# imazen/codec-eval

Measured on AMD Instinct MI355X. Metric: metric MP/s (SSIMULACRA2+DSSIM+Butteraugli) at 1/2/4/8 GPU; HBM-roofline %, higher is better.
Workload: dtype f32

## Files before the change

### codec-eval_amd/csrc/butteraugli.hip

```cpp
#include <algorithm>
#include <cmath>
#include <cstdlib>
#include <type_traits>

#include "ce_internal.h"

namespace {

constexpr int TPB = 256;
constexpr int PSY = 10;
enum { UHF0 = 0, UHF1, HF0, HF1, MF0, MF1, MF2, LF0, LF1, LF2 };

struct geom {
    uint32_t w, h, pitch;
    size_t plane;
};

struct blur_kernel {
    int len;
    float k[40];
    float lo[16], hi[16];
};

#define BA_XY                                                           \
    const uint32_t x = blockIdx.x * 64 + (threadIdx.x & 63);            \
    const uint32_t y = blockIdx.y * 4 + (threadIdx.x >> 6);             \
    if (x >= g.w || y >= g.h) return;                                   \
    const size_t o = (size_t)y * g.pitch + x

__device__ __forceinline__ uint32_t slot_of(uint32_t z, uint32_t n_refs_used, uint32_t max_refs)
{
    return z < n_refs_used ? z : max_refs + (z - n_refs_used);
}

struct plane_sel {
    uint32_t per_unit, first, n;
};

__device__ __forceinline__ uint32_t mirror(int x, int n)
{
    while (x < 0 || x >= n) x = x < 0 ? -x - 1 : 2 * n - 1 - x;
    return (uint32_t)x;
}

constexpr int BW_OUT = 8;

#ifndef CE_BA_BLUR_FMA
#define CE_BA_BLUR_FMA 0
#endif
__device__ __forceinline__ float blur_tap(float sum, float v, float k)
{
#if CE_BA_BLUR_FMA
    return __builtin_fmaf(v, k, sum);
#else
    return sum + v * k;
#endif
}

template <int LEN>
__device__ __forceinline__ float border_scale(const blur_kernel &bk, int pos, int n, float inv_wsum)
{
    constexpr int off = LEN / 2;
    if (pos - off >= 0 && pos + off <= n - 1) return inv_wsum;
    if (n >= LEN) {
        const int d = pos < off ? pos : n - 1 - pos;
        float s = 0.0f;
#pragma unroll
        for (int i = 0; i < off; i++) s = d == i ? (pos < off ? bk.lo[i] : bk.hi[i]) : s;
        return s;
    }
    float weight = 0.0f;
    for (int j = max(pos - off, 0); j <= min(pos + off, n - 1); j++) weight += bk.k[j - pos + off];
    return 1.0f / weight;
}

typedef float ba_f2 __attribute__((ext_vector_type(2)));
#ifndef CE_BH_TILES
#define CE_BH_TILES 4
#endif
constexpr int BH_TILES = CE_BH_TILES;

template <int LEN>
__global__ __launch_bounds__(TPB) void k_ba_blur_h(const float *__restrict__ in, float *__restrict__ out, geom g, plane_sel si,
                                                   plane_sel so, blur_kernel bk, float inv_wsum, uint32_t n_refs_used,
                                                   uint32_t max_refs, int by_slot, uint32_t z0)
{
    constexpr int off = LEN / 2, TW = 256, TR = 8, LEFT = 16, RAW = TW + 2 * LEFT, ROWF = RAW + RAW / 8 + 1, SH = LEFT - off;
    static_assert(off <= LEFT, "tile halo");
    __shared__ float tile[TR * ROWF];
    const uint32_t u = blockIdx.z / si.n + z0, k = blockIdx.z % si.n;
    const uint32_t unit = by_slot ? slot_of(u, n_refs_used, max_refs) : u;
    const float *p = in + ((size_t)unit * si.per_unit + si.first + k) * g.plane;
    const int x0 = blockIdx.x * TW;
    constexpr int NF = (TR * (RAW / 4) + TPB - 1) / TPB;
    float4 pf[NF];
    auto fetch = [&](int y0) {
#pragma unroll
        for (int m = 0; m < NF; m++) {
            const int i = m * TPB + (int)threadIdx.x, r = i / (RAW / 4), c = 4 * (i % (RAW / 4)), gx = x0 - LEFT + c, gy = y0 + r;
            float4 v = make_float4(0.0f, 0.0f, 0.0f, 0.0f);
            if (r < TR && gx >= 0 && gx < (int)g.pitch && gy < (int)g.h) {
                v = *reinterpret_cast<const float4 *>(p + (size_t)gy * g.pitch + gx);
                if (gx + 3 >= (int)g.w) {
                    if (gx + 0 >= (int)g.w) v.x = 0.0f;
                    if (gx + 1 >= (int)g.w) v.y = 0.0f;
                    if (gx + 2 >= (int)g.w) v.z = 0.0f;
                    v.w = 0.0f;
                }
            }
            pf[m] = v;
        }
    };
    const int r = threadIdx.x >> 5, cx = threadIdx.x & 31, gx0 = x0 + 8 * cx;
    __shared__ __attribute__((aligned(16))) float s_scale[TW];
    {
        const int gx = x0 + (int)threadIdx.x;
        s_scale[threadIdx.x] = gx < (int)g.w ? border_scale<LEN>(bk, gx, (int)g.w, inv_wsum) : 0.0f;
    }
    constexpr int NV = BW_OUT + LEN - 1, NP = (NV + 1) / 2;
    const float *row = &tile[r * ROWF + 9 * cx];
    auto at = [&](int j) { return row[(j + SH) + ((j + SH) >> 3)]; };
    const int y_first = blockIdx.y * (TR * BH_TILES);
    fetch(y_first);
#pragma unroll 1
    for (int t = 0; t < BH_TILES; t++) {
        const int y0 = y_first + t * TR;
        if (y0 >= (int)g.h) break;
        if (t) __syncthreads();
#pragma unroll
        for (int m = 0; m < NF; m++) {
            const int i = m * TPB + (int)threadIdx.x, rr = i / (RAW / 4), c = 4 * (i % (RAW / 4));
            if (rr < TR) {
                float *tp = &tile[rr * ROWF + c + (c >> 3)];
                tp[0] = pf[m].x, tp[1] = pf[m].y, tp[2] = pf[m].z, tp[3] = pf[m].w;
            }
        }
        if (t + 1 < BH_TILES && y0 + TR < (int)g.h) fetch(y0 + TR);
        __syncthreads();
        const int gy = y0 + r;
        if (gy >= (int)g.h || gx0 >= (int)g.w) continue;
        ba_f2 pe[NP], po[NP];
#pragma unroll
        for (int i = 0; i < NP; i++) {
            pe[i] = ba_f2{at(2 * i), 2 * i + 1 < NV ? at(2 * i + 1) : 0.0f};
            po[i] = ba_f2{2 * i + 1 < NV ? at(2 * i + 1) : 0.0f, 2 * i + 2 < NV ? at(2 * i + 2) : 0.0f};
        }
        float *dst = out + ((size_t)unit * so.per_unit + so.first + k) * g.plane + (size_t)gy * g.pitch + gx0;
        float res[BW_OUT];
#pragma unroll
        for (int op = 0; op < BW_OUT / 2; op++) {
            ba_f2 sum = {0.0f, 0.0f};
#pragma unroll
            for (int j = 0; j < LEN; j++) {
                const int idx = 2 * op + j;
                const ba_f2 src = (idx & 1) ? po[idx >> 1] : pe[idx >> 1];
#if CE_BA_BLUR_FMA
                sum = __builtin_elementwise_fma(src, ba_f2{bk.k[j], bk.k[j]}, sum);
#else
                const ba_f2 prod = src * ba_f2{bk.k[j], bk.k[j]};
                sum = sum + prod;
#endif
            }
            res[2 * op] = sum.x * s_scale[8 * cx + 2 * op];
            res[2 * op + 1] = sum.y * s_scale[8 * cx + 2 * op + 1];
        }
        if (gx0 + BW_OUT <= (int)g.w) {
            *reinterpret_cast<float4 *>(dst) = make_float4(res[0], res[1], res[2], res[3]);
            *reinterpret_cast<float4 *>(dst + 4) = make_float4(res[4], res[5], res[6], res[7]);
        } else {
#pragma unroll
            for (int o = 0; o < BW_OUT; o++)
                if (gx0 + o < (int)g.w) dst[o] = res[o];
        }
    }
}

__device__ __forceinline__ void opsin_absorbance(float in0, float in1, float in2, float &o0, float &o1, float &o2)
{
    const float mixi0 = 0.29956550340058319f, mixi1 = 0.63373087833825936f, mixi2 = 0.077705617820981968f, mixi3 = 1.7557483643287353f;
    const float mixi4 = 0.22158691104574774f, mixi5 = 0.69391388044116142f, mixi6 = 0.0987313588422f, mixi7 = 1.7557483643287353f;
    const float mixi8 = 0.02f, mixi9 = 0.02f, mixi10 = 0.20480129041026129f, mixi11 = 12.226454707163354f;
    o0 = __builtin_fmaf(mixi0, in0, __builtin_fmaf(mixi1, in1, __builtin_fmaf(mixi2, in2, mixi3)));
    o1 = __builtin_fmaf(mixi4, in0, __builtin_fmaf(mixi5, in1, __builtin_fmaf(mixi6, in2, mixi7)));
    o2 = __builtin_fmaf(mixi8, in0, __builtin_fmaf(mixi9, in1, __builtin_fmaf(mixi10, in2, mixi11)));
}

__device__ __forceinline__ float fast_log2f(float x)
{
    const float p0 = -1.8503833400518310E-06f, p1 = 1.4287160470083755E+00f, p2 = 7.4245873327820566E-01f;
    const float q0 = 9.9032814277590719E-01f, q1 = 1.0096718572241148E+00f, q2 = 1.7409343003366853E-01f;
    const int32_t xb = (int32_t)__float_as_uint(x);
    const int32_t es = (xb - 0x3f2aaaab) >> 23;
    const float m = __uint_as_float((uint32_t)xb - ((uint32_t)es << 23));
    const float t = m - 1.0f;
    const float yp = __builtin_fmaf(__builtin_fmaf(p2, t, p1), t, p0);
    const float yq = __builtin_fmaf(__builtin_fmaf(q2, t, q1), t, q0);
    return ce_div_noscale(yp, yq) + (float)es;
}

__device__ __forceinline__ float gamma_f(float v)
{
    const float kRetMul = 19.245013259874995f * 0.693147180559945f, kRetAdd = -23.16046239805755f;
    if (v < 0.0f) v = 0.0f;
    const float biased = v + 9.9710635769299145f;
    return __builtin_fmaf(kRetMul, fast_log2f(biased), kRetAdd);
}

constexpr int FT = 32, FR = FT + 4;
template <typename T>
__device__ __forceinline__ float ba_linear_of(const float *tab, T v) { return tab[v]; }
template <>
__device__ __forceinline__ float ba_linear_of<float>(const float *, float v) { return v; }

template <bool HALF, typename T>
__global__ __launch_bounds__(TPB) void k_ba_front(const uint8_t *__restrict__ refs, const uint8_t *__restrict__ tests,
                                                  const float *__restrict__ lut, const float *__restrict__ lut_test, geom gi,
                                                  float *__restrict__ xyb, geom g, float w0, float w1, float w2,
                                                  float intensity_target, size_t img_bytes, uint32_t n_refs_used, uint32_t max_refs,
                                                  uint32_t z0)
{
    __shared__ float L[3][FR * FR];
    __shared__ float H[3][FR * FT];
    constexpr bool U8 = sizeof(T) == 1;
    __shared__ float s_lut[256];
    if (U8) s_lut[threadIdx.x] = lut[threadIdx.x];
    const uint32_t z = blockIdx.z + z0, slot = slot_of(z, n_refs_used, max_refs);
    const int w = (int)g.w, h = (int)g.h, x0 = blockIdx.x * FT, y0 = blockIdx.y * FT, gx0 = x0 - 2, gy0 = y0 - 2;
    const uint8_t *src8 = z < n_refs_used ? refs + (size_t)z * img_bytes : tests + (size_t)(z - n_refs_used) * img_bytes;
    const T *srcT = reinterpret_cast<const T *>(src8);
    const float *tab = U8 ? s_lut : (z < n_refs_used ? lut : lut_test);
    const int W8 = HALF ? (int)gi.w : w, H8 = HALF ? (int)gi.h : h;
    __syncthreads();
    const bool interior = gx0 >= 0 && gy0 >= 0 && gx0 + FR <= w && gy0 + FR <= h;
    auto load12 = [&](const uint8_t *p, uint32_t &v0, uint32_t &v1, uint32_t &v2) {
        const uintptr_t a = reinterpret_cast<uintptr_t>(p);
        const uint32_t *q = reinterpret_cast<const uint32_t *>(a & ~(uintptr_t)3);
        const uint32_t d0 = q[0], d1 = q[1], d2 = q[2], d3 = q[3], sh = (uint32_t)(a & 3);
        v0 = __builtin_amdgcn_alignbyte(d1, d0, sh), v1 = __builtin_amdgcn_alignbyte(d2, d1, sh), v2 = __builtin_amdgcn_alignbyte(d3, d2, sh);
    };
    if (U8 && !HALF && interior) {
        for (int i = threadIdx.x; i < FR * (FR / 4); i += TPB) {
            const int ly = i / (FR / 4), lx = 4 * (i % (FR / 4));
            uint32_t v0, v1, v2;
            load12(src8 + ((size_t)(gy0 + ly) * w + gx0 + lx) * 3, v0, v1, v2);
            const int o = ly * FR + lx;
            L[0][o] = s_lut[v0 & 255u], L[1][o] = s_lut[(v0 >> 8) & 255u], L[2][o] = s_lut[(v0 >> 16) & 255u];
            L[0][o + 1] = s_lut[v0 >> 24], L[1][o + 1] = s_lut[v1 & 255u], L[2][o + 1] = s_lut[(v1 >> 8) & 255u];
            L[0][o + 2] = s_lut[(v1 >> 16) & 255u], L[1][o + 2] = s_lut[v1 >> 24], L[2][o + 2] = s_lut[v2 & 255u];
            L[0][o + 3] = s_lut[(v2 >> 8) & 255u], L[1][o + 3] = s_lut[(v2 >> 16) & 255u], L[2][o + 3] = s_lut[v2 >> 24];
        }
    } else if (U8 && HALF && interior && 2 * (gx0 + FR) <= W8 && 2 * (gy0 + FR) <= H8) {
        for (int i = threadIdx.x; i < FR * (FR / 2); i += TPB) {
            const int ly = i / (FR / 2), lx = 2 * (i % (FR / 2));
            uint32_t a0, a1, a2, b0, b1, b2;
            const uint8_t *p = src8 + ((size_t)(2 * (gy0 + ly)) * W8 + 2 * (gx0 + lx)) * 3;
            load12(p, a0, a1, a2);
            load12(p + (size_t)W8 * 3, b0, b1, b2);
            const int o = ly * FR + lx;
#define CE_Q(v) (0.25f * s_lut[(v)])
            L[0][o] = ((0.0f + CE_Q(a0 & 255u)) + CE_Q(a0 >> 24)) + CE_Q(b0 & 255u) + CE_Q(b0 >> 24);
            L[1][o] = ((0.0f + CE_Q((a0 >> 8) & 255u)) + CE_Q(a1 & 255u)) + CE_Q((b0 >> 8) & 255u) + CE_Q(b1 & 255u);
            L[2][o] = ((0.0f + CE_Q((a0 >> 16) & 255u)) + CE_Q((a1 >> 8) & 255u)) + CE_Q((b0 >> 16) & 255u) + CE_Q((b1 >> 8) & 255u);
            L[0][o + 1] = ((0.0f + CE_Q((a1 >> 16) & 255u)) + CE_Q((a2 >> 8) & 255u)) + CE_Q((b1 >> 16) & 255u) + CE_Q((b2 >> 8) & 255u);
            L[1][o + 1] = ((0.0f + CE_Q(a1 >> 24)) + CE_Q((a2 >> 16) & 255u)) + CE_Q(b1 >> 24) + CE_Q((b2 >> 16) & 255u);
            L[2][o + 1] = ((0.0f + CE_Q(a2 & 255u)) + CE_Q(a2 >> 24)) + CE_Q(b2 & 255u) + CE_Q(b2 >> 24);
#undef CE_Q
        }
    } else
    for (int i = threadIdx.x; i < FR * FR; i += TPB) {
        const int lx = i % FR, ly = i / FR, X = gx0 + lx, Y = gy0 + ly;
        if (X >= 0 && X < w && Y >= 0 && Y < h) {
            if (!HALF) {
                const T *px = srcT + ((size_t)Y * w + X) * 3;
                L[0][i] = ba_linear_of<T>(tab, px[0]);
                L[1][i] = ba_linear_of<T>(tab, px[1]);
                L[2][i] = ba_linear_of<T>(tab, px[2]);
            } else {
                float acc[3] = {0.0f, 0.0f, 0.0f};
#pragma unroll
                for (int dy = 0; dy < 2; dy++)
#pragma unroll
                    for (int dx = 0; dx < 2; dx++) {
                        const int ix = 2 * X + dx, iy = 2 * Y + dy;
                        if (ix < W8 && iy < H8) {
                            const T *px = srcT + ((size_t)iy * W8 + ix) * 3;
#pragma unroll
                            for (int c = 0; c < 3; c++) acc[c] += 0.25f * ba_linear_of<T>(tab, px[c]);
                        }
                    }
#pragma unroll
                for (int c = 0; c < 3; c++) {
                    float v = acc[c];
                    if ((W8 & 1) && X == w - 1) v *= 2.0f;
                    if ((H8 & 1) && Y == h - 1) v *= 2.0f;
                    L[c][i] = v;
                }
            }
        }
    }
    __syncthreads();
    auto stages = [&](auto in_tag) {
        constexpr bool IN = decltype(in_tag)::value;
        for (int i = threadIdx.x; i < FR * FT; i += TPB) {
            const int tx = i % FT, ly = i / FT, X = x0 + tx, Y = gy0 + ly;
            if (IN || (X < w && Y >= 0 && Y < h)) {
                const int c0 = X - gx0;
                const int m1 = IN ? c0 - 1 : (int)mirror(X - 1, w) - gx0, p1 = IN ? c0 + 1 : (int)mirror(X + 1, w) - gx0,
                          m2 = IN ? c0 - 2 : (int)mirror(X - 2, w) - gx0, p2 = IN ? c0 + 2 : (int)mirror(X + 2, w) - gx0;
    #pragma unroll
                for (int c = 0; c < 3; c++) {
                    const float *r = &L[c][ly * FR];
                    H[c][i] = r[c0] * w0 + (r[m1] + r[p1]) * w1 + (r[m2] + r[p2]) * w2;
                }
            }
        }
        __syncthreads();
        for (int i = threadIdx.x; i < FT * FT; i += TPB) {
            const int tx = i % FT, ty = i / FT, X = x0 + tx, Y = y0 + ty;
            if (!IN && (X >= w || Y >= h)) continue;
            const int r0 = Y - gy0;
            const int rm1 = IN ? r0 - 1 : (int)mirror(Y - 1, h) - gy0, rp1 = IN ? r0 + 1 : (int)mirror(Y + 1, h) - gy0,
                      rm2 = IN ? r0 - 2 : (int)mirror(Y - 2, h) - gy0, rp2 = IN ? r0 + 2 : (int)mirror(Y + 2, h) - gy0;
            float bl[3], ln[3];
    #pragma unroll
            for (int c = 0; c < 3; c++) {
                const float *col = &H[c][tx];
                bl[c] = col[r0 * FT] * w0 + (col[rm1 * FT] + col[rp1 * FT]) * w1 + (col[rm2 * FT] + col[rp2 * FT]) * w2;
                ln[c] = L[c][(ty + 2) * FR + tx + 2];
            }
            const float mn = 1e-4f;
            float p0, p1v, p2v;
            opsin_absorbance(bl[0] * intensity_target, bl[1] * intensity_target, bl[2] * intensity_target, p0, p1v, p2v);
            p0 = p0 > mn ? p0 : mn;
            p1v = p1v > mn ? p1v : mn;
            p2v = p2v > mn ? p2v : mn;
            float s0 = ce_div_noscale(gamma_f(p0), p0), s1 = ce_div_noscale(gamma_f(p1v), p1v), s2 = ce_div_noscale(gamma_f(p2v), p2v);
            s0 = s0 > mn ? s0 : mn;
            s1 = s1 > mn ? s1 : mn;
            s2 = s2 > mn ? s2 : mn;
            float c0, c1, c2;
            opsin_absorbance(ln[0] * intensity_target, ln[1] * intensity_target, ln[2] * intensity_target, c0, c1, c2);
            c0 *= s0;
            c1 *= s1;
            c2 *= s2;
            const float min01 = 1.7557483643287353f, min2 = 12.226454707163354f;
            c0 = c0 > min01 ? c0 : min01;
            c1 = c1 > min01 ? c1 : min01;
            c2 = c2 > min2 ? c2 : min2;
            const size_t o = (size_t)slot * 3 * g.plane + (size_t)Y * g.pitch + X;
            xyb[o] = c0 - c1;
            xyb[o + g.plane] = c0 + c1;
            xyb[o + 2 * g.plane] = c2;
        }
    };
    if (interior)
        stages(std::true_type{});
    else
        stages(std::false_type{});
}

__device__ __forceinline__ float remove_range(float w, float x) { return x > w ? x - w : (x < -w ? x + w : 0.0f); }
__device__ __forceinline__ float amplify_range(float w, float x) { return x > w ? x + w : (x < -w ? x - w : x + x); }
__device__ __forceinline__ float maximum_clamp(float v, float maxval)
{
    const float kMul = 0.724216145665f;
    if (v >= maxval) return __builtin_fmaf(v - maxval, kMul, maxval);
    if (v < -maxval) return __builtin_fmaf(v + maxval, kMul, -maxval);
    return v;
}

enum { EPI_LF = 0, EPI_MF = 1, EPI_HF = 2, EPI_MASK = 3 };

__device__ __forceinline__ float mask_pre_one(float uhf0, float hf0, float uhf1, float hf1)
{
    const float muls[3] = {2.5f, 0.4f, 0.4f};
    const float xdiff = (uhf0 + hf0) * muls[0];
    const float ydiff = uhf1 * muls[1] + hf1 * muls[2];
    const float m = sqrtf(xdiff * xdiff + ydiff * ydiff);
    const float kMul = 6.19424080439f, kBias = 12.61050594197f;
    const float bias = kMul * kBias;
    const float sqrt_bias = sqrtf(bias);
    return sqrtf(kMul * fabsf(m) + bias) - sqrt_bias;
}

template <int LEN, int EPI, bool HV, int TR>
__global__ __launch_bounds__(TPB) void k_ba_blur_v_split(const float *__restrict__ tmp, const float *__restrict__ xyb,
                                                         float *__restrict__ psy, geom g, blur_kernel bk, float inv_wsum,
                                                         uint32_t n_refs_used, uint32_t max_refs, uint32_t z0,
                                                         float *__restrict__ mask_in, float *__restrict__ aux_out)
{
    constexpr int NP = EPI == EPI_HF ? 2 : EPI == EPI_MASK ? 1 : 3;
    constexpr int off = LEN / 2, TW = 64, PARTS = TR / 32, RAW = TR + LEN - 1;
    static_assert(TR % 32 == 0, "four waves x 8 rows per part");
    constexpr int LEFT = off <= 4 ? 4 : 8, IW = HV ? TW + 2 * LEFT : TW;
    static_assert(!HV || off <= LEFT, "row-pass halo");
    __shared__ __attribute__((aligned(16))) float tile[RAW * TW];
    __shared__ __attribute__((aligned(16))) float in_t[HV ? RAW * IW : 4];
    const uint32_t slot = slot_of(blockIdx.z + z0, n_refs_used, max_refs);
    const int x0 = blockIdx.x * TW, y0 = blockIdx.y * TR;
    const int c = threadIdx.x & 63, wv = threadIdx.x >> 6, gx = x0 + c;
    const bool col_live = gx < (int)g.w;
    float res[NP][PARTS][BW_OUT];
    constexpr int NF = (RAW * (IW / 4) + TPB - 1) / TPB;
    float4 pf[NF];
    auto fetch = [&](int q) {
        const float *p = tmp + (EPI == EPI_MASK ? (size_t)slot : (size_t)slot * 3 + q) * g.plane;
#pragma unroll
        for (int m = 0; m < NF; m++) {
            const int i = m * TPB + (int)threadIdx.x, r = i / (IW / 4), X = x0 - (HV ? LEFT : 0) + 4 * (i % (IW / 4)), Y = y0 - off + r;
            float4 v = make_float4(0.f, 0.f, 0.f, 0.f);
            if (r < RAW && Y >= 0 && Y < (int)g.h && X >= 0 && X < (int)g.pitch) v = *reinterpret_cast<const float4 *>(p + (size_t)Y * g.pitch + X);
            v.x = X < (int)g.w ? v.x : 0.0f;
            v.y = X + 1 < (int)g.w ? v.y : 0.0f;
            v.z = X + 2 < (int)g.w ? v.z : 0.0f;
            v.w = X + 3 < (int)g.w ? v.w : 0.0f;
            pf[m] = v;
        }
    };
    auto stash = [&]() {
#pragma unroll
        for (int m = 0; m < NF; m++) {
            const int i = m * TPB + (int)threadIdx.x;
            if (i < RAW * (IW / 4)) *reinterpret_cast<float4 *>((HV ? in_t : tile) + 4 * i) = pf[m];
        }
    };
    constexpr int S0 = LEFT - off, NW = (S0 + 3 + LEN + 3) / 4;
    const int rc4 = 4 * ((int)threadIdx.x % (TW / 4));
    __shared__ __attribute__((aligned(16))) float s_sx[HV ? TW : 4];
    if (HV && threadIdx.x < TW)
        s_sx[threadIdx.x] = x0 + (int)threadIdx.x < (int)g.w ? border_scale<LEN>(bk, x0 + (int)threadIdx.x, (int)g.w, inv_wsum) : 0.0f;
    float scale_x[4] = {0.0f, 0.0f, 0.0f, 0.0f};
    fetch(0);
    if (HV) {
        stash();
        __syncthreads();
#pragma unroll
        for (int k = 0; k < 4; k++) scale_x[k] = s_sx[rc4 + k];
    }
#pragma unroll
    for (int q = 0; q < NP; q++) {
        if (HV) {
#pragma unroll 1
            for (int u = threadIdx.x; u < RAW * (TW / 4); u += TPB) {
                const int r = u / (TW / 4);
                const float4 *src = reinterpret_cast<const float4 *>(in_t + r * IW + rc4);
                float wnd[4 * NW];
#pragma unroll
                for (int m = 0; m < NW; m++) {
                    const float4 v = src[m];
                    wnd[4 * m] = v.x, wnd[4 * m + 1] = v.y, wnd[4 * m + 2] = v.z, wnd[4 * m + 3] = v.w;
                }
                float out[4];
#pragma unroll
                for (int k = 0; k < 4; k++) {
                    float sum = 0.0f;
#pragma unroll
                    for (int j = 0; j < LEN; j++) sum = blur_tap(sum, wnd[S0 + k + j], bk.k[j]);
                    out[k] = sum * scale_x[k];
                }
                *reinterpret_cast<float4 *>(tile + r * TW + rc4) = make_float4(out[0], out[1], out[2], out[3]);
            }
            __syncthreads();
            if (q + 1 < NP) fetch(q + 1);
        } else {
            if (q) __syncthreads();
            stash();
            if (q + 1 < NP) fetch(q + 1);
            __syncthreads();
        }
#pragma unroll
        for (int part = 0; part < PARTS; part++) {
            const int ly = 32 * part + 8 * wv, gy0 = y0 + ly;
            if (col_live && gy0 < (int)g.h) {
                float v[BW_OUT + LEN - 1];
#pragma unroll
                for (int j = 0; j < BW_OUT + LEN - 1; j++) v[j] = tile[(ly + j) * TW + c];
#pragma unroll
                for (int o = 0; o < BW_OUT; o++) {
                    float sum = 0.0f;
#pragma unroll
                    for (int j = 0; j < LEN; j++) sum = blur_tap(sum, v[o + j], bk.k[j]);
                    res[q][part][o] = sum * border_scale<LEN>(bk, gy0 + o, (int)g.h, inv_wsum);
                }
            }
        }
        if (HV && q + 1 < NP) {
            stash();
            __syncthreads();
        }
    }
    if (!col_live) return;
    const size_t pl = g.plane;
#pragma unroll
    for (int part = 0; part < PARTS; part++) {
        const int gy0 = y0 + 32 * part + 8 * wv;
        if (gy0 >= (int)g.h) break;
        float *ps = psy + (size_t)slot * PSY * g.plane + (size_t)gy0 * g.pitch + gx;
#pragma unroll
        for (int o = 0; o < BW_OUT; o++) {
            if (gy0 + o >= (int)g.h) break;
            float *q = ps + (size_t)o * g.pitch;
            const size_t ao = (size_t)slot * 3 * pl + (size_t)(gy0 + o) * g.pitch + gx;
            if (EPI == EPI_LF) {
                const float *xs = xyb + (size_t)slot * 3 * pl + (size_t)(gy0 + o) * g.pitch + gx;
                const float lx = res[0][part][o], ly = res[1][part][o], lb = res[2][part][o];
                aux_out[ao] = xs[0] - lx;
                aux_out[ao + pl] = xs[pl] - ly;
                aux_out[ao + 2 * pl] = xs[2 * pl] - lb;
                const float xmul = 33.832837186260f, ymul = 14.458268100570f, bmul = 49.87984651440f, y_to_b_mul = -0.362267051518f;
                const float bb = __builtin_fmaf(y_to_b_mul, ly, lb);
                q[LF2 * pl] = bb * bmul;
                q[LF0 * pl] = lx * xmul;
                q[LF1 * pl] = ly * ymul;
            } else if (EPI == EPI_MF) {
                const float kRemoveMfRange = 0.29f, kAddMfRange = 0.1f;
                const float mf0 = res[0][part][o], mf1 = res[1][part][o];
                const float hf0 = tmp[ao] - mf0, hf1 = tmp[ao + pl] - mf1;
                q[MF0 * pl] = remove_range(kRemoveMfRange, mf0);
                q[MF1 * pl] = amplify_range(kAddMfRange, mf1);
                q[MF2 * pl] = res[2][part][o];
                const float suppress = 46.0f, sv = 0.653020556257f, one_minus_s = 1.0f - 0.653020556257f;
                const float scaler = __builtin_fmaf(suppress / __builtin_fmaf(hf1, hf1, suppress), one_minus_s, sv);
                aux_out[ao] = scaler * hf0;
                aux_out[ao + pl] = hf1;
            } else if (EPI == EPI_MASK) {
                aux_out[(size_t)slot * pl + (size_t)(gy0 + o) * g.pitch + gx] = res[0][part][o];
            } else {
                const float kRemoveHfRange = 1.5f, kAddHfRange = 0.132f, kRemoveUhfRange = 0.04f;
                const float kMaxclampHf = 28.4691806922f, kMaxclampUhf = 5.19175294647f, kMulYHf = 2.155f, kMulYUhf = 2.69313763794f;
                float hf0_out, uhf0_out, hf1_out, uhf1_out;
                {
                    const float hf = res[0][part][o];
                    const float uhf = tmp[ao] - hf;
                    hf0_out = remove_range(kRemoveHfRange, hf);
                    uhf0_out = remove_range(kRemoveUhfRange, uhf);
                    q[HF0 * pl] = hf0_out;
                    q[UHF0 * pl] = uhf0_out;
                }
                {
                    float hf = maximum_clamp(res[1][part][o], kMaxclampHf);
                    float uhf = tmp[ao + pl] - hf;
                    uhf = maximum_clamp(uhf, kMaxclampUhf);
                    uhf *= kMulYUhf;
                    uhf1_out = uhf;
                    q[UHF1 * pl] = uhf;
                    hf *= kMulYHf;
                    hf1_out = amplify_range(kAddHfRange, hf);
                    q[HF1 * pl] = hf1_out;
                }
                mask_in[(size_t)slot * pl + (size_t)(gy0 + o) * g.pitch + gx] = mask_pre_one(uhf0_out, hf0_out, uhf1_out, hf1_out);
            }
        }
    }
}

struct malta_params {
    float norm2_0gt1, norm2_0lt1, norm1;
};

struct mline {
    int n;
    signed char d[9][2];
};

__device__ constexpr mline MALTA_HF[16] = {
    {9, {{-4, 0}, {-3, 0}, {-2, 0}, {-1, 0}, {0, 0}, {1, 0}, {2, 0}, {3, 0}, {4, 0}}},
    {9, {{0, -4}, {0, -3}, {0, -2}, {0, -1}, {0, 0}, {0, 1}, {0, 2}, {0, 3}, {0, 4}}},
    {7, {{-3, -3}, {-2, -2}, {-1, -1}, {0, 0}, {1, 1}, {2, 2}, {3, 3}}},
    {7, {{3, -3}, {2, -2}, {1, -1}, {0, 0}, {-1, 1}, {-2, 2}, {-3, 3}}},
    {9, {{1, -4}, {1, -3}, {1, -2}, {0, -1}, {0, 0}, {0, 1}, {-1, 2}, {-1, 3}, {-1, 4}}},
    {9, {{-1, -4}, {-1, -3}, {-1, -2}, {0, -1}, {0, 0}, {0, 1}, {1, 2}, {1, 3}, {1, 4}}},
    {9, {{-4, -1}, {-3, -1}, {-2, -1}, {-1, 0}, {0, 0}, {1, 0}, {2, 1}, {3, 1}, {4, 1}}},
    {9, {{-4, 1}, {-3, 1}, {-2, 1}, {-1, 0}, {0, 0}, {1, 0}, {2, -1}, {3, -1}, {4, -1}}},
    {7, {{-2, -3}, {-1, -2}, {-1, -1}, {0, 0}, {1, 1}, {1, 2}, {2, 3}}},
    {7, {{2, -3}, {1, -2}, {1, -1}, {0, 0}, {-1, 1}, {-1, 2}, {-2, 3}}},
    {7, {{-3, -2}, {-2, -1}, {-1, -1}, {0, 0}, {1, 1}, {2, 1}, {3, 2}}},
    {7, {{3, -2}, {2, -1}, {1, -1}, {0, 0}, {-1, 1}, {-2, 1}, {-3, 2}}},
    {8, {{-4, 2}, {-3, 2}, {-2, 1}, {-1, 1}, {0, 0}, {1, 0}, {2, -1}, {3, -1}}},
    {8, {{-4, -2}, {-3, -2}, {-2, -1}, {-1, -1}, {0, 0}, {1, 0}, {2, 1}, {3, 1}}},
    {8, {{-2, -4}, {-2, -3}, {-1, -2}, {-1, -1}, {0, 0}, {0, 1}, {1, 2}, {1, 3}}},
    {8, {{2, -4}, {2, -3}, {1, -2}, {1, -1}, {0, 0}, {0, 1}, {-1, 2}, {-1, 3}}},
};
__device__ constexpr mline MALTA_LF[16] = {
    {5, {{-4, 0}, {-2, 0}, {0, 0}, {2, 0}, {4, 0}}},
    {5, {{0, -4}, {0, -2}, {0, 0}, {0, 2}, {0, 4}}},
    {5, {{-3, -3}, {-2, -2}, {0, 0}, {2, 2}, {3, 3}}},
    {5, {{3, -3}, {2, -2}, {0, 0}, {-2, 2}, {-3, 3}}},
    {5, {{1, -4}, {1, -2}, {0, 0}, {-1, 2}, {-1, 4}}},
    {5, {{-1, -4}, {-1, -2}, {0, 0}, {1, 2}, {1, 4}}},
    {5, {{-4, -1}, {-2, -1}, {0, 0}, {2, 1}, {4, 1}}},
    {5, {{-4, 1}, {-2, 1}, {0, 0}, {2, -1}, {4, -1}}},
    {5, {{-2, -3}, {-1, -2}, {0, 0}, {1, 2}, {2, 3}}},
    {5, {{2, -3}, {1, -2}, {0, 0}, {-1, 2}, {-2, 3}}},
    {5, {{-3, -2}, {-2, -1}, {0, 0}, {2, 1}, {3, 2}}},
    {5, {{3, -2}, {2, -1}, {0, 0}, {-2, 1}, {-3, 2}}},
    {5, {{-4, 2}, {-2, 1}, {0, 0}, {2, -1}, {4, -2}}},
    {5, {{-4, -2}, {-2, -1}, {0, 0}, {2, 1}, {4, 2}}},
    {5, {{-2, -4}, {-1, -2}, {0, 0}, {1, 2}, {2, 4}}},
    {5, {{2, -4}, {1, -2}, {0, 0}, {-1, 2}, {-2, 4}}},
};

constexpr int MT = 64, MH = 4, ML = MT + 2 * MH;

__device__ constexpr bool malta_line_descends(const mline &ln)
{
    for (int j = 1; j < ln.n; j++)
        if (ln.d[j][1] > ln.d[j - 1][1]) return false;
    return ln.d[0][1] != ln.d[ln.n - 1][1];
}
__device__ constexpr bool malta_line_monotone(const mline &ln)
{
    bool up = true, down = true;
    for (int j = 1; j < ln.n; j++) {
        if (ln.d[j][1] < ln.d[j - 1][1]) up = false;
        if (ln.d[j][1] > ln.d[j - 1][1]) down = false;
    }
    return up || down;
}
__device__ constexpr bool malta_tables_monotone()
{
    for (int k = 0; k < 16; k++)
        if (!malta_line_monotone(MALTA_HF[k]) || !malta_line_monotone(MALTA_LF[k])) return false;
    return true;
}
static_assert(malta_tables_monotone(), "the row-streaming Malta unit needs every line's rows to be visited in one direction");

struct malta_bands {
    malta_params p[2][3];
};

__device__ __forceinline__ void div2_shared_rcp(float a0, float a1, float b, float &q0, float &q1)
{
    const float r = ce_rcp_refined(b);
    q0 = ce_div_refined(a0, b, r);
    q1 = ce_div_refined(a1, b, r);
}

__device__ __forceinline__ float malta_pre_diff(float v0, float v1, const malta_params &mp)
{
    const float absval = 0.5f * (fabsf(v0) + fabsf(v1));
    const float diff = v0 - v1;
    float scaler, scaler2;
    div2_shared_rcp(mp.norm2_0gt1, mp.norm2_0lt1, mp.norm1 + absval, scaler, scaler2);
    const float r = scaler * diff;
    const float fabs0 = fabsf(v0), too_small = 0.55f * fabs0, too_big = 1.05f * fabs0;
    const bool neg = v0 < 0;
    const float u = neg ? -v1 : v1;
    const bool lo = u < too_small, hi = u > too_big;
    const float impact = scaler2 * (lo ? too_small - u : u - too_big);
    const float rn = r + ((neg == lo) ? -impact : impact);
    return (lo || hi) ? rn : r;
}

__device__ __forceinline__ float l2_asym_acc(float total, float val0, float val1, float vw_0gt1, float vw_0lt1)
{
    const float diff = val0 - val1;
    total = __builtin_fmaf(diff * diff, vw_0gt1, total);
    const float fabs0 = fabsf(val0);
    const float too_small = 0.4f * fabs0, too_big = fabs0;
    const float if_neg = val1 > -too_small ? val1 + too_small : (val1 < -too_big ? -val1 - too_big : 0.0f);
    const float if_pos = val1 < too_small ? too_small - val1 : (val1 > too_big ? val1 - too_big : 0.0f);
// ... 621 lines not shown
```

Baseline: 20610.

## Use packed loads on border tiles and pre-fill mirrored halo in butteraugli front

Border tiles of the butteraugli XYB front-end kernel now use the packed 12-byte u8 loads per group wherever the window stays inside the image, falling back to per-pixel loads only at the edges. After loading, the out-of-image halo cells in shared memory are filled from their mirrored sources, so the separable blur stages run a single branch-free path with fixed offsets instead of computing mirror indices per tap. This is meant to cut the divergent, slower handling of edge tiles. In exchange it adds an extra fill pass and barrier on border tiles and more complex load selection logic.

```diff
diff --git a/codec-eval_amd/csrc/ba_front_geom.h b/codec-eval_amd/csrc/ba_front_geom.h
--- /dev/null
+++ b/codec-eval_amd/csrc/ba_front_geom.h
@@ -0,0 +1,63 @@
+#pragma once
+
+#include <cstddef>
+#include <cstdint>
+
+inline constexpr int ba_front_tile = 32, ba_front_halo = 2, ba_front_region = ba_front_tile + 2 * ba_front_halo;
+inline constexpr int ba_front_groups4 = ba_front_region / 4, ba_front_groups2 = ba_front_region / 2;
+
+constexpr int ba_mirror(int x, int n)
+{
+    while (x < 0 || x >= n) x = x < 0 ? -x - 1 : 2 * n - 1 - x;
+    return x;
+}
+
+constexpr int ba_front_shift4(int gx0, int w) { return (gx0 < 0 || gx0 + ba_front_region > w) ? ba_front_halo : 0; }
+constexpr bool ba_front_group4_contiguous(int g, int shift) { return shift == 0 || g < ba_front_groups4 - 1; }
+constexpr int ba_front_group4_cell(int g, int k, int shift)
+{
+    return ba_front_group4_contiguous(g, shift) ? shift + 4 * g + k : (k < 2 ? k : ba_front_region - 4 + k);
+}
+constexpr void ba_front_task2(int i, int &lx, int &ly) { ly = i / ba_front_groups2, lx = 2 * (i % ba_front_groups2); }
+
+constexpr bool ba_front_window_inside(size_t off, uint32_t mis, size_t bytes)
+{
+    const size_t first = (mis + off) & ~(size_t)3;
+    return first >= mis && first + 16 <= mis + bytes;
+}
+
+constexpr bool ba_front_fast4(int X0, int Y, int w, int h, uint32_t mis)
+{
+    if (Y < 0 || Y >= h || X0 < 0 || X0 + 4 > w) return false;
+    return ba_front_window_inside(((size_t)Y * w + X0) * 3, mis, (size_t)w * h * 3);
+}
+
+constexpr bool ba_front_fast2_half(int X0, int Y, int W8, int H8, uint32_t mis)
+{
+    if (Y < 0 || 2 * Y + 1 >= H8 || X0 < 0 || 2 * X0 + 3 >= W8) return false;
+    const size_t off = ((size_t)(2 * Y) * W8 + 2 * X0) * 3, bytes = (size_t)W8 * H8 * 3;
+    return ba_front_window_inside(off, mis, bytes) && ba_front_window_inside(off + (size_t)W8 * 3, mis, bytes);
+}
+
+constexpr bool ba_front_all_fast4(int gx0, int gy0, int w, int h, uint32_t mis)
+{
+    return ba_front_fast4(gx0, gy0, w, h, mis) && ba_front_fast4(gx0 + ba_front_region - 4, gy0 + ba_front_region - 1, w, h, mis);
+}
+constexpr bool ba_front_all_fast2_half(int gx0, int gy0, int W8, int H8, uint32_t mis)
+{
+    return ba_front_fast2_half(gx0, gy0, W8, H8, mis) &&
+           ba_front_fast2_half(gx0 + ba_front_region - 2, gy0 + ba_front_region - 1, W8, H8, mis);
+}
+
+constexpr int ba_front_out_lo(int g0) { return g0 < 0 ? -g0 : 0; }
+constexpr int ba_front_out_hi(int g0, int n) { return n - g0 < ba_front_region ? n - g0 : ba_front_region; }
+constexpr int ba_front_out_line(int k, int lo, int hi) { return k < lo ? k : hi + (k - lo); }
+
+enum { BA_RIM_IMAGE = 0, BA_RIM_COPY = 1, BA_RIM_ZERO = 2 };
+constexpr int ba_front_rim(int X, int Y, int w, int h, int gx0, int gy0, int &src)
+{
+    if (X >= 0 && X < w && Y >= 0 && Y < h) return BA_RIM_IMAGE;
+    if (X < -ba_front_halo || X >= w + ba_front_halo || Y < -ba_front_halo || Y >= h + ba_front_halo) return BA_RIM_ZERO;
+    src = (ba_mirror(Y, h) - gy0) * ba_front_region + (ba_mirror(X, w) - gx0);
+    return BA_RIM_COPY;
+}
diff --git a/codec-eval_amd/csrc/butteraugli.hip b/codec-eval_amd/csrc/butteraugli.hip
--- a/codec-eval_amd/csrc/butteraugli.hip
+++ b/codec-eval_amd/csrc/butteraugli.hip
@@ -3,6 +3,7 @@
 #include <cstdlib>
 #include <type_traits>
 
+#include "ba_front_geom.h"
 #include "ce_internal.h"
 
 namespace {
@@ -36,12 +37,6 @@
 struct plane_sel {
     uint32_t per_unit, first, n;
 };
-
-__device__ __forceinline__ uint32_t mirror(int x, int n)
-{
-    while (x < 0 || x >= n) x = x < 0 ? -x - 1 : 2 * n - 1 - x;
-    return (uint32_t)x;
-}
 
 constexpr int BW_OUT = 8;
 
@@ -232,15 +227,46 @@
     const int W8 = HALF ? (int)gi.w : w, H8 = HALF ? (int)gi.h : h;
     __syncthreads();
     const bool interior = gx0 >= 0 && gy0 >= 0 && gx0 + FR <= w && gy0 + FR <= h;
+    const uint32_t mis = (uint32_t)(reinterpret_cast<uintptr_t>(src8) & 3);
     auto load12 = [&](const uint8_t *p, uint32_t &v0, uint32_t &v1, uint32_t &v2) {
         const uintptr_t a = reinterpret_cast<uintptr_t>(p);
         const uint32_t *q = reinterpret_cast<const uint32_t *>(a & ~(uintptr_t)3);
         const uint32_t d0 = q[0], d1 = q[1], d2 = q[2], d3 = q[3], sh = (uint32_t)(a & 3);
         v0 = __builtin_amdgcn_alignbyte(d1, d0, sh), v1 = __builtin_amdgcn_alignbyte(d2, d1, sh), v2 = __builtin_amdgcn_alignbyte(d3, d2, sh);
     };
-    if (U8 && !HALF && interior) {
-        for (int i = threadIdx.x; i < FR * (FR / 4); i += TPB) {
-            const int ly = i / (FR / 4), lx = 4 * (i % (FR / 4));
+    auto load_cell = [&](int lx, int ly) {
+        const int i = ly * FR + lx, X = gx0 + lx, Y = gy0 + ly;
+        if (X >= 0 && X < w && Y >= 0 && Y < h) {
+            if (!HALF) {
+                const T *px = srcT + ((size_t)Y * w + X) * 3;
+                L[0][i] = ba_linear_of<T>(tab, px[0]);
+                L[1][i] = ba_linear_of<T>(tab, px[1]);
+                L[2][i] = ba_linear_of<T>(tab, px[2]);
+            } else {
+                float acc[3] = {0.0f, 0.0f, 0.0f};
+#pragma unroll
+                for (int dy = 0; dy < 2; dy++)
+#pragma unroll
+                    for (int dx = 0; dx < 2; dx++) {
+                        const int ix = 2 * X + dx, iy = 2 * Y + dy;
+                        if (ix < W8 && iy < H8) {
+                            const T *px = srcT + ((size_t)iy * W8 + ix) * 3;
+#pragma unroll
+                            for (int c = 0; c < 3; c++) acc[c] += 0.25f * ba_linear_of<T>(tab, px[c]);
+                        }
+                    }
+#pragma unroll
+                for (int c = 0; c < 3; c++) {
+                    float v = acc[c];
+                    if ((W8 & 1) && X == w - 1) v *= 2.0f;
+                    if ((H8 & 1) && Y == h - 1) v *= 2.0f;
+                    L[c][i] = v;
+                }
+            }
+        }
+    };
+    if (U8 && !HALF) {
+        auto packed4 = [&](int lx, int ly) {
             uint32_t v0, v1, v2;
             load12(src8 + ((size_t)(gy0 + ly) * w + gx0 + lx) * 3, v0, v1, v2);
             const int o = ly * FR + lx;
@@ -248,10 +274,21 @@
             L[0][o + 1] = s_lut[v0 >> 24], L[1][o + 1] = s_lut[v1 & 255u], L[2][o + 1] = s_lut[(v1 >> 8) & 255u];
             L[0][o + 2] = s_lut[(v1 >> 16) & 255u], L[1][o + 2] = s_lut[v1 >> 24], L[2][o + 2] = s_lut[v2 & 255u];
             L[0][o + 3] = s_lut[(v2 >> 8) & 255u], L[1][o + 3] = s_lut[(v2 >> 16) & 255u], L[2][o + 3] = s_lut[v2 >> 24];
-        }
-    } else if (U8 && HALF && interior && 2 * (gx0 + FR) <= W8 && 2 * (gy0 + FR) <= H8) {
-        for (int i = threadIdx.x; i < FR * (FR / 2); i += TPB) {
-            const int ly = i / (FR / 2), lx = 2 * (i % (FR / 2));
+        };
+        if (ba_front_all_fast4(gx0, gy0, w, h, mis)) {
+            for (int i = threadIdx.x; i < FR * ba_front_groups4; i += TPB) packed4(4 * (i % ba_front_groups4), i / ba_front_groups4);
+        } else {
+            const int shift = ba_front_shift4(gx0, w);
+            for (int i = threadIdx.x; i < FR * ba_front_groups4; i += TPB) {
+                const int g = i % ba_front_groups4, ly = i / ba_front_groups4, lx = ba_front_group4_cell(g, 0, shift);
+                if (ba_front_group4_contiguous(g, shift) && ba_front_fast4(gx0 + lx, gy0 + ly, w, h, mis))
+                    packed4(lx, ly);
+                else
+                    for (int k = 0; k < 4; k++) load_cell(ba_front_group4_cell(g, k, shift), ly);
+            }
+        }
+    } else if (U8 && HALF) {
+        auto packed2 = [&](int lx, int ly) {
             uint32_t a0, a1, a2, b0, b1, b2;
             const uint8_t *p = src8 + ((size_t)(2 * (gy0 + ly)) * W8 + 2 * (gx0 + lx)) * 3;
             load12(p, a0, a1, a2);
@@ -265,98 +302,86 @@
             L[1][o + 1] = ((0.0f + CE_Q(a1 >> 24)) + CE_Q((a2 >> 16) & 255u)) + CE_Q(b1 >> 24) + CE_Q((b2 >> 16) & 255u);
             L[2][o + 1] = ((0.0f + CE_Q(a2 & 255u)) + CE_Q(a2 >> 24)) + CE_Q(b2 & 255u) + CE_Q(b2 >> 24);
 #undef CE_Q
-        }
-    } else
-    for (int i = threadIdx.x; i < FR * FR; i += TPB) {
-        const int lx = i % FR, ly = i / FR, X = gx0 + lx, Y = gy0 + ly;
-        if (X >= 0 && X < w && Y >= 0 && Y < h) {
-            if (!HALF) {
-                const T *px = srcT + ((size_t)Y * w + X) * 3;
-                L[0][i] = ba_linear_of<T>(tab, px[0]);
-                L[1][i] = ba_linear_of<T>(tab, px[1]);
-                L[2][i] = ba_linear_of<T>(tab, px[2]);
-            } else {
-                float acc[3] = {0.0f, 0.0f, 0.0f};
-#pragma unroll
-                for (int dy = 0; dy < 2; dy++)
-#pragma unroll
-                    for (int dx = 0; dx < 2; dx++) {
-                        const int ix = 2 * X + dx, iy = 2 * Y + dy;
-                        if (ix < W8 && iy < H8) {
-                            const T *px = srcT + ((size_t)iy * W8 + ix) * 3;
-#pragma unroll
-                            for (int c = 0; c < 3; c++) acc[c] += 0.25f * ba_linear_of<T>(tab, px[c]);
-                        }
-                    }
-#pragma unroll
-                for (int c = 0; c < 3; c++) {
-                    float v = acc[c];
-                    if ((W8 & 1) && X == w - 1) v *= 2.0f;
-                    if ((H8 & 1) && Y == h - 1) v *= 2.0f;
-                    L[c][i] = v;
+        };
+        if (ba_front_all_fast2_half(gx0, gy0, W8, H8, mis)) {
+            for (int i = threadIdx.x; i < FR * ba_front_groups2; i += TPB) packed2(2 * (i % ba_front_groups2), i / ba_front_groups2);
+        } else {
+            for (int i = threadIdx.x; i < FR * ba_front_groups2; i += TPB) {
+                int lx, ly;
+                ba_front_task2(i, lx, ly);
+                if (ba_front_fast2_half(gx0 + lx, gy0 + ly, W8, H8, mis)) {
+                    packed2(lx, ly);
+                } else {
+                    load_cell(lx, ly);
+                    load_cell(lx + 1, ly);
                 }
             }
         }
+    } else {
+        for (int i = threadIdx.x; i < FR * FR; i += TPB) load_cell(i % FR, i / FR);
     }
     __syncthreads();
-    auto stages = [&](auto in_tag) {
-        constexpr bool IN = decltype(in_tag)::value;
-        for (int i = threadIdx.x; i < FR * FT; i += TPB) {
-            const int tx = i % FT, ly = i / FT, X = x0 + tx, Y = gy0 + ly;
-            if (IN || (X < w && Y >= 0 && Y < h)) {
-                const int c0 = X - gx0;
-                const int m1 = IN ? c0 - 1 : (int)mirror(X - 1, w) - gx0, p1 = IN ? c0 + 1 : (int)mirror(X + 1, w) - gx0,
-                          m2 = IN ? c0 - 2 : (int)mirror(X - 2, w) - gx0, p2 = IN ? c0 + 2 : (int)mirror(X + 2, w) - gx0;
-    #pragma unroll
-                for (int c = 0; c < 3; c++) {
-                    const float *r = &L[c][ly * FR];
-                    H[c][i] = r[c0] * w0 + (r[m1] + r[p1]) * w1 + (r[m2] + r[p2]) * w2;
-                }
-            }
+    if (!interior) {
+        auto fill = [&](int lx, int ly) {
+            const int i = ly * FR + lx;
+            int src = 0;
+            if (ba_front_rim(gx0 + lx, gy0 + ly, w, h, gx0, gy0, src) == BA_RIM_COPY)
+                L[0][i] = L[0][src], L[1][i] = L[1][src], L[2][i] = L[2][src];
+            else
+                L[0][i] = 0.0f, L[1][i] = 0.0f, L[2][i] = 0.0f;
+        };
+        const int xlo = ba_front_out_lo(gx0), xhi = ba_front_out_hi(gx0, w), ylo = ba_front_out_lo(gy0), yhi = ba_front_out_hi(gy0, h);
+        for (int t = threadIdx.x; t < (xlo + FR - xhi) * FR; t += TPB) fill(ba_front_out_line(t / FR, xlo, xhi), t % FR);
+        for (int t = threadIdx.x; t < (ylo + FR - yhi) * FR; t += TPB) {
+            const int lx = t % FR;
+            if (lx >= xlo && lx < xhi) fill(lx, ba_front_out_line(t / FR, ylo, yhi));
         }
         __syncthreads();
-        for (int i = threadIdx.x; i < FT * FT; i += TPB) {
-            const int tx = i % FT, ty = i / FT, X = x0 + tx, Y = y0 + ty;
-            if (!IN && (X >= w || Y >= h)) continue;
-            const int r0 = Y - gy0;
-            const int rm1 = IN ? r0 - 1 : (int)mirror(Y - 1, h) - gy0, rp1 = IN ? r0 + 1 : (int)mirror(Y + 1, h) - gy0,
-                      rm2 = IN ? r0 - 2 : (int)mirror(Y - 2, h) - gy0, rp2 = IN ? r0 + 2 : (int)mirror(Y + 2, h) - gy0;
-            float bl[3], ln[3];
-    #pragma unroll
-            for (int c = 0; c < 3; c++) {
-                const float *col = &H[c][tx];
-                bl[c] = col[r0 * FT] * w0 + (col[rm1 * FT] + col[rp1 * FT]) * w1 + (col[rm2 * FT] + col[rp2 * FT]) * w2;
-                ln[c] = L[c][(ty + 2) * FR + tx + 2];
-            }
-            const float mn = 1e-4f;
-            float p0, p1v, p2v;
-            opsin_absorbance(bl[0] * intensity_target, bl[1] * intensity_target, bl[2] * intensity_target, p0, p1v, p2v);
-            p0 = p0 > mn ? p0 : mn;
-            p1v = p1v > mn ? p1v : mn;
-            p2v = p2v > mn ? p2v : mn;
-            float s0 = ce_div_noscale(gamma_f(p0), p0), s1 = ce_div_noscale(gamma_f(p1v), p1v), s2 = ce_div_noscale(gamma_f(p2v), p2v);
-            s0 = s0 > mn ? s0 : mn;
-            s1 = s1 > mn ? s1 : mn;
-            s2 = s2 > mn ? s2 : mn;
-            float c0, c1, c2;
-            opsin_absorbance(ln[0] * intensity_target, ln[1] * intensity_target, ln[2] * intensity_target, c0, c1, c2);
-            c0 *= s0;
-            c1 *= s1;
-            c2 *= s2;
-            const float min01 = 1.7557483643287353f, min2 = 12.226454707163354f;
-            c0 = c0 > min01 ? c0 : min01;
-            c1 = c1 > min01 ? c1 : min01;
-            c2 = c2 > min2 ? c2 : min2;
-            const size_t o = (size_t)slot * 3 * g.plane + (size_t)Y * g.pitch + X;
-            xyb[o] = c0 - c1;
-            xyb[o + g.plane] = c0 + c1;
-            xyb[o + 2 * g.plane] = c2;
-        }
-    };
-    if (interior)
-        stages(std::true_type{});
-    else
-        stages(std::false_type{});
+    }
+    for (int i = threadIdx.x; i < FR * FT; i += TPB) {
+        const int tx = i % FT, ly = i / FT, c0 = tx + 2;
+#pragma unroll
+        for (int c = 0; c < 3; c++) {
+            const float *r = &L[c][ly * FR];
+            H[c][i] = r[c0] * w0 + (r[c0 - 1] + r[c0 + 1]) * w1 + (r[c0 - 2] + r[c0 + 2]) * w2;
+        }
+    }
+    __syncthreads();
+    for (int i = threadIdx.x; i < FT * FT; i += TPB) {
+        const int tx = i % FT, ty = i / FT, X = x0 + tx, Y = y0 + ty;
+        if (X >= w || Y >= h) continue;
+        const int r0 = ty + 2;
+        float bl[3], ln[3];
+#pragma unroll
+        for (int c = 0; c < 3; c++) {
+            const float *col = &H[c][tx];
+            bl[c] = col[r0 * FT] * w0 + (col[(r0 - 1) * FT] + col[(r0 + 1) * FT]) * w1 + (col[(r0 - 2) * FT] + col[(r0 + 2) * FT]) * w2;
+            ln[c] = L[c][(ty + 2) * FR + tx + 2];
+        }
+        const float mn = 1e-4f;
+        float p0, p1v, p2v;
+        opsin_absorbance(bl[0] * intensity_target, bl[1] * intensity_target, bl[2] * intensity_target, p0, p1v, p2v);
+        p0 = p0 > mn ? p0 : mn;
+        p1v = p1v > mn ? p1v : mn;
+        p2v = p2v > mn ? p2v : mn;
+        float s0 = ce_div_noscale(gamma_f(p0), p0), s1 = ce_div_noscale(gamma_f(p1v), p1v), s2 = ce_div_noscale(gamma_f(p2v), p2v);
+        s0 = s0 > mn ? s0 : mn;
+        s1 = s1 > mn ? s1 : mn;
+        s2 = s2 > mn ? s2 : mn;
+        float c0, c1, c2;
+        opsin_absorbance(ln[0] * intensity_target, ln[1] * intensity_target, ln[2] * intensity_target, c0, c1, c2);
+        c0 *= s0;
+        c1 *= s1;
+        c2 *= s2;
+        const float min01 = 1.7557483643287353f, min2 = 12.226454707163354f;
+        c0 = c0 > min01 ? c0 : min01;
+        c1 = c1 > min01 ? c1 : min01;
+        c2 = c2 > min2 ? c2 : min2;
+        const size_t o = (size_t)slot * 3 * g.plane + (size_t)Y * g.pitch + X;
+        xyb[o] = c0 - c1;
+        xyb[o + g.plane] = c0 + c1;
+        xyb[o + 2 * g.plane] = c2;
+    }
 }
 
 __device__ __forceinline__ float remove_range(float w, float x) { return x > w ? x - w : (x < -w ? x + w : 0.0f); }
```

Measured after the change: 20890, median of 6. +1.3%, better.
